# edegens/ptype

Hardware: AMD Instinct MI355X
Metric: messages/sec (higher is better)
Workload: dtype int64; 1 GPU; model=calculator actor (Calculator.Multiply), global_batch=8388608, parallelism=actors sharded over 1 GPU(s), actors=131072, chunks=1, wire=v2, record_bytes=20, reply_bytes=9, client_batch=SoA (actor u32, A i64, B i64), hip_graph=True, steps_per_graph=1, placement=random, delivery=mailbox, mailbox_slots=131072, mailbox_ring_bytes=1344380288, mailbox_record_bytes=8

## Files before the change

### ptype_amd/csrc/hip/mailbox_sort.hip

```cpp
#include "mailbox_sort_dev.hpp"

namespace ptype {

template <int MODE>
__global__ __launch_bounds__(kST) void mbx_count_kernel(SortIn in, uint32_t log_s, uint32_t* __restrict__ hist,
                                                        uint32_t* __restrict__ gsum, uint32_t* __restrict__ rw) {
  __shared__ uint32_t cnt[kMboxSortMaxShards];
  const uint32_t S = 1u << log_s;
  const uint32_t v = virt_block(blockIdx.x, in.G);
  for (uint32_t s = threadIdx.x; s < S; s += kST) cnt[s] = 0;
  __syncthreads();
  const uint32_t t0 = v * in.tpb, t1 = min(t0 + in.tpb, in.tiles);
  uint32_t a[kSK];
  if (t0 < t1) load_actors(in, t0, a);
  for (uint32_t t = t0; t < t1; ++t) {
    int r[kSK];
    uint32_t mb[kSK];
    resolve_k<MODE>(in, a, r, mb);
    if (t + 1 < t1) load_actors(in, t + 1, a);
#pragma unroll
    for (int k = 0; k < kSK; ++k) {
      const int64_t i = tile_index(t, k);
      const bool ok = r[k] == in.rank_self && mb[k] < kMaxMbox;
      if (i < in.M) rw[i] = ok ? mb[k] : kNoSlot;
// ... 108 lines not shown
      }
      const uint32_t off = wcnt(w, sh[k]) + wr[k];
      if (off >= room[sh[k]]) {
        if (spill) {
          ++n_spill;
          sidx[i] = kSpillSlot;
          continue;
        }
        ++n_ovf;
        if (wsidx) sidx[i] = kNoSlot;
        write_status(rv, origin, kStatusOverflow);
        continue;
      }
      const int64_t x0 = v0[k], x1 = v1[k], x2 = v2[k];
      const uint32_t mt = meth[k];
      const uint64_t slot = slot_at(mv, sh[k], base[sh[k]] + off);
      if (wsidx) sidx[i] = (uint32_t)slot;
      if (mt < 128u && fits_i32(x0) && fits_i32(x1) && x2 == 0) {
        *reinterpret_cast<u32x4*>(rec_a(mv, slot)) =
            u32x4{origin | kCompactMark, mb[k] | (mt << 24), (uint32_t)x0, (uint32_t)x1};
      } else {
        const uint32_t fl = x2 != 0 ? (uint32_t)kFlagA2 : 0u;
        *reinterpret_cast<u32x4*>(rec_a(mv, slot)) =
            u32x4{origin | kCompactMark, mb[k] | kCompactLong, (mt & 0xffffu) | (fl << 16), 0u};
        *reinterpret_cast<u32x4*>(rec_b(mv, slot)) =
            u32x4{(uint32_t)x0, (uint32_t)((uint64_t)x0 >> 32), (uint32_t)x1, (uint32_t)((uint64_t)x1 >> 32)};
        if (fl) mv.a2[slot] = x2;
      }
      ++n_enq;
    }
    if (tinfo) {
      for (uint32_t s = threadIdx.x; s < S; s += kST) {
        const uint32_t r0 = wcnt(0, s), rr = run[s];
        const uint32_t cc = r0 >= room[s] ? 0u : min(rr - r0, room[s] - r0);
        tinfo[(size_t)t * 2 * S + s] = (uint32_t)(base[s] + r0) + shard_rot(mv, s);
        tinfo[(size_t)t * 2 * S + S + s] = cc | (rr > room[s] ? kRunSpilled : 0u);
      }
    }
    __syncthreads();
  }
  block_add_stats(mv.stats, n_enq, kMbEnqueued, n_ovf, kMbOverflow, n_miss, kMbNoActor);
  if (spill) {
    __syncthreads();
    block_add_stats(mv.stats, n_spill, kMbSpilled, 0, -1, 0, -1);
  }
}

template <int = 0>
__global__ __launch_bounds__(256) void mbx_presence_kernel(const uint8_t* __restrict__ dirr, uint32_t n_dir,
                                                           int rank_self, uint32_t* __restrict__ pres) {
  const uint32_t wi = blockIdx.x * 256u + threadIdx.x;
  if (wi >= pres_words(n_dir)) return;
  alignas(16) uint8_t b[16];
  if (wi * 16 + 16 <= n_dir) {
    *reinterpret_cast<uint4*>(b) = *reinterpret_cast<const uint4*>(dirr + (size_t)wi * 16);
  } else {
#pragma unroll
    for (uint32_t j = 0; j < 16; ++j) b[j] = wi * 16 + j < n_dir ? dirr[wi * 16 + j] : kRankMissing;
  }
  uint32_t w = 0;
#pragma unroll
  for (uint32_t j = 0; j < 16; ++j) {
    const uint32_t st = b[j] == (uint8_t)rank_self ? 1u : b[j] == kRankFallback ? 2u : 0u;
    w |= st << (2 * j);
  }
  pres[wi] = w;
}

template <int MODE, bool A2, bool MC>
__global__ __launch_bounds__(kST) void mbx_onesweep_kernel(SortIn in, MboxView mv, unsigned long long* __restrict__ desc,
                                                           unsigned* __restrict__ tctr, uint32_t* __restrict__ gsum,
                                                           uint32_t* __restrict__ sidx, uint32_t* __restrict__ tinfo,
                                                           uint32_t* __restrict__ rw, ReplyView rv, bool spill,
                                                           bool all_sidx, bool reserve) {
  extern __shared__ __align__(16) unsigned char smem_os[];
  (void)onesweep_tile<MODE, A2, MC>(in, mv, desc, tctr, gsum, sidx, tinfo, rw, rv, spill, all_sidx, smem_os, reserve);
}

__host__ __device__ constexpr size_t persist_lds_bytes(uint32_t S) {
  return (size_t)S * (8 + 4 + 2 * 4 + 2 * 4 * (kST / kWave));
}

template <int = 0>
__global__ __launch_bounds__(kST) void mbx_persist_sort_kernel(SortIn in, MboxView mv, uint32_t* __restrict__ sidx,
                                                               uint32_t* __restrict__ tinfo, uint32_t* __restrict__ rw,
                                                               ReplyView rv) {
  constexpr int SK = kSK;
  extern __shared__ __align__(16) unsigned char smem_ps[];
  const uint32_t S = 1u << mv.log_s;
  unsigned long long* base = reinterpret_cast<unsigned long long*>(smem_ps);
  uint32_t* room = reinterpret_cast<uint32_t*>(base + S);
  uint32_t* pre2 = room + S;
  uint32_t* wcnt2 = pre2 + 2 * S;
  uint32_t* lpres = reinterpret_cast<uint32_t*>(smem_ps + ((persist_lds_bytes(S) + 15) & ~(size_t)15));
  __shared__ uint32_t tmax[3];
  __shared__ uint32_t vote[2];
  const unsigned w = threadIdx.x / kWave, lane = lane_id();
  const uint32_t G = gridDim.x, T = in.tiles;
  uint32_t first = blockIdx.x, stride = G, n = blockIdx.x < T ? (T - blockIdx.x + G - 1) / G : 0u;
  if (G >= 8 && (G & 7) == 0 && (T & 7) == 0) {
    const uint32_t j = blockIdx.x >> 3, T8 = T >> 3;
    stride = G >> 3;
    first = (blockIdx.x & 7) * T8 + j;
    n = j < T8 ? (T8 - j + stride - 1) / stride : 0u;
  }
  if (n == 0) return;
  stage_pres(in, lpres);
  for (uint32_t s = threadIdx.x; s < S; s += kST) {
    uint64_t tl;
    room[s] = os_ring_room(mv, s, tl);
    base[s] = tl;
  }
  if (threadIdx.x < 3) tmax[threadIdx.x] = 0;
  if (threadIdx.x < 2) vote[threadIdx.x] = 0;
  for (uint32_t s = lane; s < S; s += kWave) wcnt2[w * S + s] = 0;
  __syncthreads();
  const uint32_t w8 = in.rec8 ? *in.r8w : 0u;
  const bool maxima = in.rec8 || in.recw;
  uint32_t n_enq = 0, n_ovf = 0, n_miss = 0, n_spill = 0;
  uint32_t nx[SK];
  int64_t v0[SK], v1[SK];
  PackedRanks<SK> wrp;
  {
    uint32_t a[SK], wr[SK];
    int r[SK];
    const bool full = tile_is_full<SK>(in, first);
    load_actors<SK>(in, first, a);
    load_args_tile<SK>(in, first, full, v0, v1);
    os_resolve<4, SK>(in, lpres, a, r, nx);
    os_rank<SK>(in, mv.log_s, first, r, nx, wcnt2 + w * S, wr);
#pragma unroll
    for (int k = 0; k < SK / 2; ++k) wrp.p[k] = wr[2 * k] | (wr[2 * k + 1] << 16);
  }
  __syncthreads();
  uint32_t rc = 0, rx = 0;
  if (threadIdx.x < S) {
    rc = os_wave_offsets(wcnt2, S, threadIdx.x);
    rx = os_reserve(mv, threadIdx.x, rc);
  }
  for (uint32_t it = 0; it < n; ++it) {
    const uint32_t t = first + it * stride, b = it & 1;
    uint32_t* pre = pre2 + b * S;
    uint32_t* wcnt_all = wcnt2 + b * (kST / kWave) * S;
    const bool full = tile_is_full<SK>(in, t);
    uint32_t mb[SK];
#pragma unroll
    for (int k = 0; k < SK; ++k) mb[k] = nx[k];
    const bool more = it + 1 < n;
    const bool full_next = more && tile_is_full<SK>(in, t + stride);
    if (more) load_actors<SK>(in, t + stride, nx);
    os_loads_in<SK>(v0, v1, nx);
    int sp = 0;
    if (threadIdx.x < S) {
      const uint32_t s = threadIdx.x;
      pre[s] = rx;
      sp = os_run_info(mv, tinfo, t, S, s, base[s], room[s], rx, rc);
    }
    const uint32_t escm = os_fields<SK>(in, w8, mb, v0, v1, tmax);
    sp |= escm != 0;
    if (__any(sp) && lane == 0) vote[b] = 1u;
    __syncthreads();
    const bool tile_spill = __builtin_amdgcn_readfirstlane((int)vote[b]) != 0;
    if (threadIdx.x == 0) {
      if (tile_spill) tinfo[(size_t)t * 2 * S + S] |= kRunSpilled;
      if (maxima) {
        (void)atomicExch(&in.r8max[t], tmax[0] | (tmax[1] << 8) | (tmax[2] << 16));
        tmax[0] = tmax[1] = tmax[2] = 0;
      }
    }
#pragma unroll
    for (int k = 0; k < SK; ++k) {
      const int64_t i = tile_index<SK>(t, k);
      if (!full && i >= in.M) continue;
      os_store_msg<SK>(in, mv, rv, i, base, room, pre, wcnt_all + w * S, mb[k], wrp[k], v0[k], v1[k], 0, in.method_uniform,
                       (escm >> k) & 1u, w8, true, tile_spill, sidx, rw, n_enq, n_ovf, n_miss, n_spill);
    }
    if (more) {
      load_args_tile<SK>(in, t + stride, full_next, v0, v1);
      uint32_t* wnext = wcnt2 + (b ^ 1) * (kST / kWave) * S;
      for (uint32_t s = lane; s < S; s += kWave) wnext[w * S + s] = 0;
      uint32_t a[SK], wr[SK];
      int r[SK];
#pragma unroll
      for (int k = 0; k < SK; ++k) a[k] = nx[k];
      os_resolve<4, SK>(in, lpres, a, r, nx);
      os_rank<SK>(in, mv.log_s, t + stride, r, nx, wnext + w * S, wr);
#pragma unroll
      for (int k = 0; k < SK / 2; ++k) wrp.p[k] = wr[2 * k] | (wr[2 * k + 1] << 16);
      __syncthreads();
      if (threadIdx.x == 0) vote[b] = 0u;
      if (threadIdx.x < S) {
        rc = os_wave_offsets(wnext, S, threadIdx.x);
        rx = os_reserve(mv, threadIdx.x, rc);
      }
    }
  }
  block_add_stats(mv.stats, n_enq, kMbEnqueued, n_ovf, kMbOverflow, n_miss, kMbNoActor);
  __syncthreads();
  block_add_stats(mv.stats, n_spill, kMbSpilled, 0, -1, 0, -1);
}

template <int FIXED>
__global__ __launch_bounds__(kST) void mbx_drain_msg_kernel(MboxView mv, SortIn in, const uint32_t* __restrict__ sidx,
                                                            const uint32_t* __restrict__ rw,
                                                            int64_t* __restrict__ state, uint32_t n_state,
                                                            uint64_t delay_ticks, OutboxView ob, ReplyView rv,
                                                            uint32_t* __restrict__ gsum, uint32_t ngroups,
                                                            unsigned* __restrict__ ticket, unsigned* __restrict__ tctr) {
  unsigned long long done = 0, failed = 0, holes = 0;
  const uint32_t v = virt_block(blockIdx.x, in.G);
  const uint32_t t0 = v * in.tpb, t1 = min(t0 + in.tpb, in.tiles);
  for (uint32_t t = t0; t < t1; ++t)
    drain_tile_msg<FIXED>(mv, in, t, sidx, rw, state, n_state, delay_ticks, ob, rv, done, failed, holes);
  block_add_stats(mv.stats, done, kMbProcessed, failed, kMbFailed, holes, kMbHoles);
  __shared__ bool last;
  if (threadIdx.x == 0) last = last_block_ticket(ticket);
  __syncthreads();
  if (last) {
    const uint32_t S = 1u << mv.log_s;
    for (uint32_t s = threadIdx.x; s < S; s += kST) epoch_commit(mv, s, epoch_sum(mv, gsum, ngroups, S, s));
    if (threadIdx.x == 0) tctr[1] += 1u;
  }
}

template <int FIXED, bool NARROW, int RF, int SK = kSK>
__global__ __launch_bounds__(kST, (NARROW && FIXED) ? 8 : 1) void mbx_drain_ring_kernel(MboxView mv, SortIn in, const uint32_t* __restrict__ tinfo,
                                                             const uint32_t* __restrict__ sidx,
                                                             const uint32_t* __restrict__ rw,
                                                             int64_t* __restrict__ state, uint32_t n_state,
                                                             uint64_t delay_ticks, OutboxView ob, ReplyView rv,
                                                             uint32_t* __restrict__ gsum, uint32_t ngroups,
                                                             unsigned* __restrict__ ticket, unsigned* __restrict__ tctr,
                                                             uint32_t* __restrict__ r8host) {
  extern __shared__ __align__(16) unsigned char smem_rd[];
  const uint32_t S = 1u << mv.log_s;
  DrainCounts dc;
  const uint32_t t = virt_block(blockIdx.x, gridDim.x);
  if (t < in.tiles)
    dc = drain_ring_tile<FIXED, NARROW, false, RF, SK>(mv, in, t, tinfo, sidx, rw, state, n_state, delay_ticks, ob,
                                                       rv, smem_rd);
  block_add_stats(mv.stats, dc.done, kMbProcessed, dc.failed, kMbFailed, dc.holes, kMbHoles);
  __shared__ bool last;
  if (threadIdx.x == 0) last = last_block_ticket(ticket);
  __syncthreads();
  if (last) {
    for (uint32_t s = threadIdx.x; s < S; s += kST) epoch_commit(mv, s, epoch_sum(mv, gsum, ngroups, S, s));
    if (threadIdx.x == 0) tctr[1] += 1u;
    if constexpr (RF != 0) rec8_next(in, const_cast<uint32_t*>(in.r8w), r8host, in.tiles);
  }
}


static const Variant<decltype(mbx_count_kernel<0>)> kCount[] = {
    MBX_ROW(vkey(0), 0, mbx_count_kernel<0>),
    MBX_ROW(vkey(1), 0, mbx_count_kernel<1>),
    MBX_ROW(vkey(2), 0, mbx_count_kernel<2>),
};
static const Variant<decltype(mbx_scatter_kernel<false, false>)> kScatter[] = {
// ... 291 lines not shown
```

### ptype_amd/csrc/hip/mailbox_sort_dev.hpp

```cpp
#pragma once
#include <algorithm>
#include <string>
#include <type_traits>
#include <vector>

#include "mailbox.hpp"
#include "mailbox_dev.hpp"
#include "route_common.hpp"
#include "sort_common.hpp"
#include "tune.hpp"

namespace ptype {

namespace {
constexpr uint32_t kCompactMark = 0x80000000u;
constexpr uint32_t kCompactLong = 0x80000000u;
}

constexpr uint32_t kNoSlot = 0xffffffffu;
constexpr uint32_t kSpillSlot = 0xfffffffeu;
constexpr uint32_t kRunSpilled = 0x80000000u;
constexpr int kWaitVmcnt0 = 0x0f70;

__host__ __device__ constexpr size_t onesweep_lds_bytes(uint32_t S) { return (size_t)S * (8 + 4 + 4 + 4 * (kST / kWave)); }
// ... 79 lines not shown
}

__device__ __forceinline__ void stage_pres(const SortIn& in, uint32_t* lpres) {
  const uint32_t nw = pres_words(in.n_dir);
  for (uint32_t w = threadIdx.x * 4; w < nw; w += blockDim.x * 4)
    *reinterpret_cast<uint4*>(lpres + w) = *reinterpret_cast<const uint4*>(in.pres + w);
}
template <int SK>
__device__ __forceinline__ void resolve_pres(const SortIn& in, const uint32_t* lpres, const uint32_t (&a)[SK],
                                             int (&r)[SK], uint32_t (&mb)[SK]) {
#pragma unroll
  for (int k = 0; k < SK; ++k) {
    mb[k] = a[k];
    if (a[k] < in.n_dir) {
      const uint32_t st = (lpres[a[k] >> 4] >> ((a[k] & 15) * 2)) & 3u;
      r[k] = st == 1 ? in.rank_self : -1;
      if (st == 2) lookup_entry(in.table, in.mask, actor_key(a[k]), r[k], mb[k]);
    } else if (a[k] != 0xffffffffu) {
      lookup_entry(in.table, in.mask, actor_key(a[k]), r[k], mb[k]);
    } else {
      r[k] = -1;
    }
  }
}

template <int MODE, int SK>
__device__ __forceinline__ void os_resolve(const SortIn& in, const uint32_t* lpres, const uint32_t (&a)[SK], int (&r)[SK],
                                           uint32_t (&mb)[SK]) {
  if constexpr (MODE == 4) resolve_pres<SK>(in, lpres, a, r, mb);
  else resolve_k<MODE, SK>(in, a, r, mb);
}

template <int SK>
__device__ __forceinline__ void os_rank(const SortIn& in, uint32_t log_s, uint32_t t, const int (&r)[SK],
                                        uint32_t (&mb)[SK], uint32_t* wrow, uint32_t (&wr)[SK]) {
  const uint32_t S = 1u << log_s;
#pragma unroll
  for (int k = 0; k < SK; ++k) {
    const bool ok = tile_index<SK>(t, k) < in.M && r[k] == in.rank_self && mb[k] < kMaxMbox;
    if (!ok) mb[k] = kNoSlot;
    const uint32_t sh = mb[k] & (S - 1);
    const uint64_t peers = match_bits(sh, log_s, __ballot(ok));
    const unsigned below = mbcnt64(peers);
    const int leader = peers ? __builtin_ctzll(peers) : 0;
    unsigned old = 0;
    if (ok && below == 0) {
      old = wrow[sh];
      wrow[sh] = old + (unsigned)__popcll(peers);
    }
    wr[k] = (unsigned)__shfl((int)old, leader) + below;
  }
}

__device__ __forceinline__ uint32_t os_wave_offsets(uint32_t* wcnt_all, uint32_t S, uint32_t s) {
  uint32_t c = 0;
#pragma unroll
  for (int ww = 0; ww < kST / kWave; ++ww) {
    const uint32_t x = wcnt_all[ww * S + s];
    wcnt_all[ww * S + s] = c;
    c += x;
  }
  return c;
}
__device__ __forceinline__ uint32_t os_reserve(const MboxView& mv, uint32_t s, uint32_t c) {
  return c ? atomicAdd(&mv.resv[s * kResvStride], c) : 0u;
}
__device__ __forceinline__ uint32_t os_ring_room(const MboxView& mv, uint32_t s, uint64_t& tl) {
  const uint64_t Q = 1ull << mv.log_q;
  tl = *ctr_tail(mv, s);
  const uint64_t hd = *ctr_head(mv, s);
  const uint64_t free = hd + Q > tl ? hd + Q - tl : 0;
  return (uint32_t)(free < 0xffffffffull ? free : 0xffffffffull);
}
__device__ __forceinline__ int os_run_info(const MboxView& mv, uint32_t* __restrict__ tinfo, uint32_t t, uint32_t S,
                                           uint32_t s, uint64_t tl, uint32_t rm, uint64_t excl, uint32_t c) {
  if (tinfo) {
    const uint32_t cc = excl >= rm ? 0u : (uint32_t)min((uint64_t)c, rm - excl);
    tinfo[(size_t)t * 2 * S + s] = (uint32_t)(tl + excl) + shard_rot(mv, s);
    tinfo[(size_t)t * 2 * S + S + s] = cc | (excl + c > rm ? kRunSpilled : 0u);
  }
  return excl + c > rm;
}

template <int SK>
__device__ __forceinline__ uint32_t os_fields(const SortIn& in, uint32_t w8, const uint32_t (&mb)[SK],
                                              const int64_t (&v0)[SK], const int64_t (&v1)[SK], uint32_t* tmax) {
  uint32_t escm = 0;
  if (!(in.rec8 || in.recw)) return escm;
  uint64_t or_m = 0, or_0 = 0, or_1 = 0;
  const uint32_t wm = w8 & 0xffu, w0 = (w8 >> 8) & 0xffu, w1 = (w8 >> 16) & 0xffu;
#pragma unroll
  for (int k = 0; k < SK; ++k) {
    if (mb[k] == kNoSlot) continue;
    const uint64_t z0 = ((uint64_t)v0[k] << 1) ^ (uint64_t)(v0[k] >> 63);
    const uint64_t z1 = ((uint64_t)v1[k] << 1) ^ (uint64_t)(v1[k] >> 63);
    or_m |= mb[k], or_0 |= z0, or_1 |= z1;
    if (in.rec8 && ((mb[k] >> wm) != 0 || (z0 >> w0) != 0 || (z1 >> w1) != 0)) escm |= 1u << k;
  }
  const uint32_t bm = wave_max_u32(bitlen64(or_m)), b0 = wave_max_u32(bitlen64(or_0)),
                 b1 = wave_max_u32(bitlen64(or_1));
  if (lane_id() == 0) {
    atomicMax(&tmax[0], bm);
    atomicMax(&tmax[1], b0);
    atomicMax(&tmax[2], b1);
  }
  return escm;
}

template <int SK>
__device__ __forceinline__ void os_loads_in(const int64_t (&v0)[SK], const int64_t (&v1)[SK], const uint32_t (&nx)[SK]) {
#pragma unroll
  for (int k = 0; k < SK; ++k) asm volatile("" ::"v"(v0[k]), "v"(v1[k]), "v"(nx[k]));
}

template <int SK>
struct PackedRanks {
  uint32_t p[SK / 2];
  __device__ __forceinline__ uint32_t operator[](int k) const { return (p[k >> 1] >> ((k & 1) * 16)) & 0xffffu; }
};

template <int SK, typename CT>
__device__ __forceinline__ void os_store_msg(const SortIn& in, const MboxView& mv, const ReplyView& rv, int64_t i,
                                             const unsigned long long* base, const uint32_t* room, const uint32_t* pre,
                                             const uint32_t* wrow, uint32_t mbk, uint32_t wrk, int64_t x0, int64_t x1,
                                             int64_t x2, uint32_t mt, bool esc, uint32_t w8, bool spill, bool wsidx,
                                             uint32_t* __restrict__ sidx, uint32_t* __restrict__ rw, CT& n_enq, CT& n_ovf,
                                             CT& n_miss, CT& n_spill) {
  const uint32_t S = 1u << mv.log_s;
  const uint32_t origin = in.origin_base + (uint32_t)i;
  if (mbk == kNoSlot) {
    ++n_miss;
    if (wsidx) sidx[i] = kNoSlot;
    write_status(rv, origin, kStatusNoActor);
    return;
  }
  const uint32_t sh = mbk & (S - 1);
  const uint32_t off = pre[sh] + wrow[sh] + wrk;
  if (off >= room[sh] || (esc && spill)) {
    if (spill) {
      ++n_spill;
      sidx[i] = kSpillSlot;
      rw[i] = mbk;
      return;
    }
    ++n_ovf;
    if (wsidx) sidx[i] = kNoSlot;
    write_status(rv, origin, kStatusOverflow);
    return;
  }
  const uint64_t slot = slot_at(mv, sh, base[sh] + off);
  if (wsidx) sidx[i] = (uint32_t)slot;
  if (in.recw) {
    *reinterpret_cast<u32x4*>(rec_a(mv, slot)) =
        u32x4{(uint32_t)x0, (uint32_t)((uint64_t)x0 >> 32), (uint32_t)x1, (uint32_t)((uint64_t)x1 >> 32)};
    rec_place(mv)[slot] = (uint16_t)(i & ((kST * SK) - 1));
  } else if (in.rec8 && esc) {
    reinterpret_cast<uint64_t*>(mv.rec)[slot] = (uint64_t)(i & ((kST * SK) - 1)) | (1ull << 63);
    *reinterpret_cast<u32x4*>(in.r8esc + 2 * slot) =
        u32x4{(uint32_t)x0, (uint32_t)((uint64_t)x0 >> 32), mbk, 0u};
  } else if (in.rec8) {
    const uint32_t wm = w8 & 0xffu, w0 = (w8 >> 8) & 0xffu;
    const uint64_t z0 = ((uint64_t)x0 << 1) ^ (uint64_t)(x0 >> 63);
    const uint64_t z1 = ((uint64_t)x1 << 1) ^ (uint64_t)(x1 >> 63);
    reinterpret_cast<uint64_t*>(mv.rec)[slot] =
        (uint64_t)(i & ((kST * SK) - 1)) | ((uint64_t)mbk << 12) | (z0 << (12 + wm)) | (z1 << (12 + wm + w0));
  } else if (mt < 128u && fits_i32(x0) && fits_i32(x1) && x2 == 0) {
    *reinterpret_cast<u32x4*>(rec_a(mv, slot)) =
        u32x4{origin | kCompactMark, mbk | (mt << 24), (uint32_t)x0, (uint32_t)x1};
  } else {
    const uint32_t fl = x2 != 0 ? (uint32_t)kFlagA2 : 0u;
    *reinterpret_cast<u32x4*>(rec_a(mv, slot)) =
        u32x4{origin | kCompactMark, mbk | kCompactLong, (mt & 0xffffu) | (fl << 16), 0u};
    *reinterpret_cast<u32x4*>(rec_b(mv, slot)) =
        u32x4{(uint32_t)x0, (uint32_t)((uint64_t)x0 >> 32), (uint32_t)x1, (uint32_t)((uint64_t)x1 >> 32)};
    if (fl) mv.a2[slot] = x2;
  }
  ++n_enq;
}

template <int MODE, bool A2, bool MC, int SK = kSK>
__device__ __forceinline__ uint32_t onesweep_tile(const SortIn& in, const MboxView& mv, unsigned long long* __restrict__ desc,
                                                  unsigned* __restrict__ tctr, uint32_t* __restrict__ gsum,
                                                  uint32_t* __restrict__ sidx, uint32_t* __restrict__ tinfo,
                                                  uint32_t* __restrict__ rw, const ReplyView& rv, bool spill,
                                                  bool all_sidx, unsigned char* smem_os, bool reserve = false) {
  const uint32_t S = 1u << mv.log_s;
  unsigned long long* base = reinterpret_cast<unsigned long long*>(smem_os);
  uint32_t* room = reinterpret_cast<uint32_t*>(base + S);
  uint32_t* pre = room + S;
  uint32_t* wcnt_all = pre + S;
  auto wcnt = [&](unsigned ww, uint32_t sh) -> uint32_t& { return wcnt_all[ww * S + sh]; };
  __shared__ uint32_t tile_s;
  __shared__ uint32_t tmax[3];
  const unsigned w = threadIdx.x / kWave, lane = lane_id();
  if (threadIdx.x < 3) tmax[threadIdx.x] = 0;
  const uint32_t tag = epoch_tag(tctr[1]);
  if (threadIdx.x == 0 && !reserve) {
    const uint32_t t = atomicAdd(&tctr[0], 1u);
    if (t == in.tiles - 1) atomicExch(&tctr[0], 0u);
    tile_s = t;
  }
  for (uint32_t s = lane; s < S; s += kWave) wcnt(w, s) = 0;
// ... 189 lines not shown
      x.a2 = in.a2 ? in.a2[i] : 0;
    } else if constexpr (RF == 1) {
      x = decode_rec8<FRESH, SK>(ha[k], in, w8, in.origin_base + t * (kST * SK));
    } else if constexpr (RF == 2) {
      x = decode_wide(ha[k], in, 0u);
    } else {
      u32x4 hb = {0u, 0u, 0u, 0u};
      int64_t a2v = 0;
      if (rec_is_long(ha[k])) {
        const u32x4* bp = reinterpret_cast<const u32x4*>(rec_b(mv, sl[k]));
        hb = FRESH ? __builtin_nontemporal_load(bp) : *bp;
        if (((ha[k].z >> 16) & kFlagA2) && mv.a2) a2v = FRESH ? __builtin_nontemporal_load(mv.a2 + sl[k]) : mv.a2[sl[k]];
      }
      x = decode_sorted(ha[k], hb, a2v);
    }
    const uint32_t origin = in.origin_base + (uint32_t)tile_index<SK>(t, k);
    if (!x.valid) {
      ++holes;
      write_status(rv, origin, kStatusNotDelivered);
      continue;
    }
    MsgRecord m;
    m.actor = x.mb;
    m.method = (uint16_t)(FIXED ? FIXED : x.method);
    m.flags = (uint16_t)x.flags;
    m.a0 = x.a0, m.a1 = x.a1, m.a2 = x.a2;
    const ReplyRecord rr = run_handler(m, state, n_state, delay_ticks, ob);
    failed += rr.status != kStatusOk;
    write_reply(rv, origin, rr);
    ++done;
  }
}

template <typename OwnT>
struct RunLds {
  uint32_t* bias;
  uint32_t* excl;
  OwnT* owner;
};

template <typename OwnT>
__device__ __forceinline__ uint32_t load_tile_runs(const MboxView& mv, const uint32_t* __restrict__ tinfo, uint32_t t,
                                                   const RunLds<OwnT>& L, int& spill) {
  __shared__ uint32_t wsum[kST / kWave];
  __shared__ uint32_t total_s;
  const uint32_t S = 1u << mv.log_s;
  const unsigned w = threadIdx.x / kWave, lane = lane_id();
  const uint32_t per = (S + kST - 1) / kST, s0 = threadIdx.x * per, s1 = min(S, s0 + per);
  uint32_t cnt[2] = {0u, 0u};
  uint32_t mine = 0;
  int sp = 0;
  for (uint32_t s = s0, q = 0; s < s1; ++s, ++q) {
    const uint32_t cw = tinfo[(size_t)t * 2 * S + S + s];
    sp |= (cw & kRunSpilled) != 0;
    cnt[q] = cw & ~kRunSpilled;
    mine += cnt[q];
    L.bias[s] = tinfo[(size_t)t * 2 * S + s];
  }
  const uint32_t incl = wave_incl_scan(mine);
  if (lane == kWave - 1) wsum[w] = incl;
  spill = __syncthreads_or(sp);
  uint32_t acc = incl - mine;
  for (unsigned ww = 0; ww < w; ++ww) acc += wsum[ww];
  if (threadIdx.x == kST - 1) total_s = acc + mine;
  for (uint32_t s = s0, q = 0; s < s1; ++s, ++q) {
    L.excl[s] = acc;
    L.bias[s] -= acc;
    for (uint32_t j = acc; j < acc + cnt[q]; ++j) L.owner[j] = (OwnT)s;
    acc += cnt[q];
  }
  __syncthreads();
  return total_s;
}

constexpr uint8_t kAbsent = 0xff;
__host__ __device__ constexpr size_t ring_drain_lds_bytes(uint32_t S, size_t tile = kSTile) {
  return S <= 256 ? tile * (8 + 1) + (size_t)S * 8 : tile * (8 + 2 + 1) + (size_t)S * 8;
}

struct DrainCounts {
  unsigned long long done = 0, failed = 0, holes = 0;
};

template <int FIXED, bool NARROW, bool FRESH, int RF = 0, int SK = kSK>
__device__ __forceinline__ DrainCounts drain_ring_tile(MboxView mv, SortIn in, uint32_t t,
                                                       const uint32_t* __restrict__ tinfo,
                                                       const uint32_t* __restrict__ sidx,
                                                       const uint32_t* __restrict__ rw, int64_t* __restrict__ state,
                                                       uint32_t n_state, uint64_t delay_ticks, OutboxView ob,
                                                       ReplyView rv, unsigned char* smem_rd) {
  unsigned long long done = 0, failed = 0, holes = 0;
  using OwnT = typename std::conditional<NARROW, uint8_t, uint16_t>::type;
  const uint32_t S = 1u << mv.log_s;
  int64_t* sval = reinterpret_cast<int64_t*>(smem_rd);
  RunLds<OwnT> L;
  L.bias = reinterpret_cast<uint32_t*>(sval + (kST * SK));
  L.excl = L.bias + S;
  L.owner = reinterpret_cast<OwnT*>(L.excl + S);
  uint8_t* sst = NARROW ? reinterpret_cast<uint8_t*>(L.owner) : reinterpret_cast<uint8_t*>(L.owner + (kST * SK));
  const uint64_t i0 = (uint64_t)t * (kST * SK);
  const uint32_t n_t = (uint32_t)min((uint64_t)(kST * SK), (uint64_t)in.M - i0);
  if constexpr (!NARROW)
    for (uint32_t j = threadIdx.x; j < (kST * SK); j += kST) sst[j] = kAbsent;
  int spill = 0;
  const uint32_t T = load_tile_runs(mv, tinfo, t, L, spill);
  if (spill) {
    drain_tile_msg<FIXED, FRESH, RF, SK>(mv, in, t, sidx, rw, state, n_state, delay_ticks, ob, rv, done, failed, holes);
    return DrainCounts{done, failed, holes};
  }
  const uint64_t sbase_mask = (1ull << mv.log_q) - 1;
  using RecT = typename std::conditional<RF == 1, uint64_t, u32x4>::type;
  const uint32_t w8 = RF == 1 ? *in.r8w : 0u;
  RecT ha[SK];
  uint32_t sl[SK];
  uint16_t pl[SK];
#pragma unroll
  for (int k = 0; k < SK; ++k) {
    const uint32_t j = (uint32_t)k * kST + threadIdx.x;
    sl[k] = kNoSlot;
    if (j < T) {
      const uint32_t s = L.owner[j];
      sl[k] = (uint32_t)(((uint64_t)s << mv.log_q) | ((L.bias[s] + j) & sbase_mask));
      if constexpr (RF == 1) {
        const uint64_t* rp = reinterpret_cast<const uint64_t*>(mv.rec) + sl[k];
        ha[k] = FRESH ? __builtin_nontemporal_load(rp) : *rp;
      } else {
        const u32x4* rp = reinterpret_cast<const u32x4*>(rec_a(mv, sl[k]));
        ha[k] = FRESH ? __builtin_nontemporal_load(rp) : *rp;
        if constexpr (RF == 2) {
          const uint16_t* pp = rec_place(mv) + sl[k];
          pl[k] = FRESH ? __builtin_nontemporal_load(pp) : *pp;
        }
      }
    }
  }
  if constexpr (NARROW) {
    __syncthreads();
    for (uint32_t j = threadIdx.x; j < (kST * SK); j += kST) sst[j] = kAbsent;
    __syncthreads();
  }
#pragma unroll
  for (int k = 0; k < SK; ++k) {
    if (sl[k] == kNoSlot) continue;
    SortRec x;
    if constexpr (RF == 1) {
      x = decode_rec8<FRESH, SK>(ha[k], in, w8, in.origin_base + (uint32_t)i0);
    } else if constexpr (RF == 2) {
      x = decode_wide(ha[k], in, in.origin_base + (uint32_t)i0 + pl[k]);
    } else {
      u32x4 hb = {0u, 0u, 0u, 0u};
      int64_t a2v = 0;
      if (rec_is_long(ha[k])) {
        const u32x4* bp = reinterpret_cast<const u32x4*>(rec_b(mv, sl[k]));
        hb = FRESH ? __builtin_nontemporal_load(bp) : *bp;
        if (((ha[k].z >> 16) & kFlagA2) && mv.a2) a2v = FRESH ? __builtin_nontemporal_load(mv.a2 + sl[k]) : mv.a2[sl[k]];
      }
      x = decode_sorted(ha[k], hb, a2v);
    }
    const uint32_t local = x.origin - in.origin_base - (uint32_t)i0;
    if (!x.valid || local >= n_t) {
      ++holes;
      continue;
    }
    MsgRecord m;
    m.actor = x.mb;
    m.method = (uint16_t)(FIXED ? FIXED : x.method);
    m.flags = (uint16_t)x.flags;
    m.a0 = x.a0, m.a1 = x.a1, m.a2 = x.a2;
    const ReplyRecord rr = run_handler(m, state, n_state, delay_ticks, ob);
    failed += rr.status != kStatusOk;
    sval[local] = rr.value;
    sst[local] = (uint8_t)rr.status;
    ++done;
  }
  __builtin_amdgcn_s_waitcnt(kWaitVmcnt0);
  __syncthreads();
  uint8_t rst[SK];
  int64_t rval[SK];
#pragma unroll
  for (int k = 0; k < SK; ++k) {
    const uint32_t j = (uint32_t)k * kST + threadIdx.x;
    rst[k] = j < n_t ? sst[j] : kAbsent;
    rval[k] = sval[j];
  }
// ... 67 lines not shown
```

Before: 65.13 billion msg/s.

## Add lean rec8 store and drain paths for small-shard stateless mailbox rings

Adds a specialized enqueue path in the persistent sort kernel for the 8-byte record case with few shards and small rings. It precomputes per-shard rotated bases, skips the general os_store_msg bookkeeping, and packs records with 32-bit zigzag shifts. On the drain side it adds a matching lean drain that resolves run slots with wave readlane instead of an LDS owner table and decodes with alignbit. It also defers the per-element escape check behind a wave-wide OR and pins the kernel to 4 waves per EU. These changes target ALU and LDS overhead per message, at the cost of much more specialized code and a possibly lower occupancy cap.

```diff
diff --git a/ptype_amd/csrc/hip/mailbox_sort.hip b/ptype_amd/csrc/hip/mailbox_sort.hip
--- a/ptype_amd/csrc/hip/mailbox_sort.hip
+++ b/ptype_amd/csrc/hip/mailbox_sort.hip
@@ -214,9 +214,9 @@
 }
 
 template <int = 0>
-__global__ __launch_bounds__(kST) void mbx_persist_sort_kernel(SortIn in, MboxView mv, uint32_t* __restrict__ sidx,
-                                                               uint32_t* __restrict__ tinfo, uint32_t* __restrict__ rw,
-                                                               ReplyView rv) {
+__global__ __launch_bounds__(kST) __attribute__((amdgpu_waves_per_eu(4, 4)))
+void mbx_persist_sort_kernel(SortIn in, MboxView mv, uint32_t* __restrict__ sidx, uint32_t* __restrict__ tinfo,
+                             uint32_t* __restrict__ rw, ReplyView rv) {
   constexpr int SK = kSK;
   extern __shared__ __align__(16) unsigned char smem_ps[];
   const uint32_t S = 1u << mv.log_s;
@@ -227,6 +227,7 @@
   uint32_t* lpres = reinterpret_cast<uint32_t*>(smem_ps + ((persist_lds_bytes(S) + 15) & ~(size_t)15));
   __shared__ uint32_t tmax[3];
   __shared__ uint32_t vote[2];
+  __shared__ uint32_t brot[kStatelessShards];
   const unsigned w = threadIdx.x / kWave, lane = lane_id();
   const uint32_t G = gridDim.x, T = in.tiles;
   uint32_t first = blockIdx.x, stride = G, n = blockIdx.x < T ? (T - blockIdx.x + G - 1) / G : 0u;
@@ -242,6 +243,7 @@
     uint64_t tl;
     room[s] = os_ring_room(mv, s, tl);
     base[s] = tl;
+    if (s < kStatelessShards) brot[s] = (uint32_t)tl + shard_rot(mv, s);
   }
   if (threadIdx.x < 3) tmax[threadIdx.x] = 0;
   if (threadIdx.x < 2) vote[threadIdx.x] = 0;
@@ -249,6 +251,8 @@
   __syncthreads();
   const uint32_t w8 = in.rec8 ? *in.r8w : 0u;
   const bool maxima = in.rec8 || in.recw;
+  const bool lean = in.rec8 && !in.recw && tinfo != nullptr && rv.slots == nullptr && S <= kStatelessShards &&
+                    rings_small(mv);
   uint32_t n_enq = 0, n_ovf = 0, n_miss = 0, n_spill = 0;
   uint32_t nx[SK];
   int64_t v0[SK], v1[SK];
@@ -288,7 +292,7 @@
       pre[s] = rx;
       sp = os_run_info(mv, tinfo, t, S, s, base[s], room[s], rx, rc);
     }
-    const uint32_t escm = os_fields<SK>(in, w8, mb, v0, v1, tmax);
+    const uint32_t escm = os_fields<SK, true>(in, w8, mb, v0, v1, tmax);
     sp |= escm != 0;
     if (__any(sp) && lane == 0) vote[b] = 1u;
     __syncthreads();
@@ -300,12 +304,36 @@
         tmax[0] = tmax[1] = tmax[2] = 0;
       }
     }
-#pragma unroll
-    for (int k = 0; k < SK; ++k) {
-      const int64_t i = tile_index<SK>(t, k);
-      if (!full && i >= in.M) continue;
-      os_store_msg<SK>(in, mv, rv, i, base, room, pre, wcnt_all + w * S, mb[k], wrp[k], v0[k], v1[k], 0, in.method_uniform,
-                       (escm >> k) & 1u, w8, true, tile_spill, sidx, rw, n_enq, n_ovf, n_miss, n_spill);
+    if (lean && !tile_spill) {
+      uint32_t* wpos = wcnt_all + w * S;
+      if (lane < S) wpos[lane] += pre[lane] + brot[lane];
+      __builtin_amdgcn_wave_barrier();
+      if (threadIdx.x < S) n_enq += rc;
+      const Rec8Fast f8 = rec8_fast(w8);
+      const uint32_t place0 = w * (SK * kWave) + lane;
+      if (f8.ok) {
+#pragma unroll
+        for (int k = 0; k < SK; ++k) {
+          const int64_t i = tile_index<SK>(t, k);
+          if (!full && i >= in.M) continue;
+          os_store_lean<SK, true>(in, mv, rv, i, place0 + k * kWave, wpos, mb[k], wrp[k], v0[k], v1[k], f8, w8, n_miss);
+        }
+      } else {
+#pragma unroll
+        for (int k = 0; k < SK; ++k) {
+          const int64_t i = tile_index<SK>(t, k);
+          if (!full && i >= in.M) continue;
+          os_store_lean<SK, false>(in, mv, rv, i, place0 + k * kWave, wpos, mb[k], wrp[k], v0[k], v1[k], f8, w8, n_miss);
+        }
+      }
+    } else {
+#pragma unroll
+      for (int k = 0; k < SK; ++k) {
+        const int64_t i = tile_index<SK>(t, k);
+        if (!full && i >= in.M) continue;
+        os_store_msg<SK>(in, mv, rv, i, base, room, pre, wcnt_all + w * S, mb[k], wrp[k], v0[k], v1[k], 0, in.method_uniform,
+                         (escm >> k) & 1u, w8, true, tile_spill, sidx, rw, n_enq, n_ovf, n_miss, n_spill);
+      }
     }
     if (more) {
       load_args_tile<SK>(in, t + stride, full_next, v0, v1);
diff --git a/ptype_amd/csrc/hip/mailbox_sort_dev.hpp b/ptype_amd/csrc/hip/mailbox_sort_dev.hpp
--- a/ptype_amd/csrc/hip/mailbox_sort_dev.hpp
+++ b/ptype_amd/csrc/hip/mailbox_sort_dev.hpp
@@ -185,7 +185,7 @@
   return excl + c > rm;
 }
 
-template <int SK>
+template <int SK, bool OR_FIRST = false>
 __device__ __forceinline__ uint32_t os_fields(const SortIn& in, uint32_t w8, const uint32_t (&mb)[SK],
                                               const int64_t (&v0)[SK], const int64_t (&v1)[SK], uint32_t* tmax) {
   uint32_t escm = 0;
@@ -198,7 +198,17 @@
     const uint64_t z0 = ((uint64_t)v0[k] << 1) ^ (uint64_t)(v0[k] >> 63);
     const uint64_t z1 = ((uint64_t)v1[k] << 1) ^ (uint64_t)(v1[k] >> 63);
     or_m |= mb[k], or_0 |= z0, or_1 |= z1;
-    if (in.rec8 && ((mb[k] >> wm) != 0 || (z0 >> w0) != 0 || (z1 >> w1) != 0)) escm |= 1u << k;
+    if constexpr (!OR_FIRST)
+      if (in.rec8 && ((mb[k] >> wm) != 0 || (z0 >> w0) != 0 || (z1 >> w1) != 0)) escm |= 1u << k;
+  }
+  if (OR_FIRST && in.rec8 && ((or_m >> wm) | (or_0 >> w0) | (or_1 >> w1)) != 0) {
+#pragma unroll
+    for (int k = 0; k < SK; ++k) {
+      if (mb[k] == kNoSlot) continue;
+      const uint64_t z0 = ((uint64_t)v0[k] << 1) ^ (uint64_t)(v0[k] >> 63);
+      const uint64_t z1 = ((uint64_t)v1[k] << 1) ^ (uint64_t)(v1[k] >> 63);
+      if ((mb[k] >> wm) != 0 || (z0 >> w0) != 0 || (z1 >> w1) != 0) escm |= 1u << k;
+    }
   }
   const uint32_t bm = wave_max_u32(bitlen64(or_m)), b0 = wave_max_u32(bitlen64(or_0)),
                  b1 = wave_max_u32(bitlen64(or_1));
@@ -221,6 +231,63 @@
   uint32_t p[SK / 2];
   __device__ __forceinline__ uint32_t operator[](int k) const { return (p[k >> 1] >> ((k & 1) * 16)) & 0xffffu; }
 };
+
+__device__ __forceinline__ bool rings_small(const MboxView& mv) { return mv.log_s + mv.log_q <= 29; }
+
+struct Rec8Fast {
+  uint32_t s0;
+  uint32_t s1h;
+  uint32_t m0;
+  uint32_t mm;
+  bool ok;
+};
+__device__ __forceinline__ Rec8Fast rec8_fast(uint32_t w8) {
+  const uint32_t wm = w8 & 0xffu, w0 = (w8 >> 8) & 0xffu, w1 = (w8 >> 16) & 0xffu;
+  Rec8Fast f;
+  f.s0 = 12 + wm;
+  f.ok = f.s0 < 32 && w0 >= 1 && w0 <= 32 && w1 <= 32 && f.s0 + w0 >= 32 && f.s0 + w0 < 64;
+  f.s1h = (f.s0 + w0) & 31u;
+  f.m0 = w0 >= 32 ? 0xffffffffu : (1u << (w0 & 31u)) - 1u;
+  f.mm = (1u << (wm & 31u)) - 1u;
+  return f;
+}
+__device__ __forceinline__ uint32_t zigzag32(int64_t x) {
+  const uint32_t lo = (uint32_t)x;
+  return (lo << 1) ^ (uint32_t)((int32_t)lo >> 31);
+}
+__device__ __forceinline__ uint64_t pack_rec8_fast(const Rec8Fast& f, uint32_t place, uint32_t mb, int64_t x0, int64_t x1) {
+  const uint32_t z0 = zigzag32(x0), z1 = zigzag32(x1);
+  const uint32_t lo = place | (mb << 12) | (z0 << f.s0);
+  const uint32_t hi = (z0 >> (32u - f.s0)) | (z1 << f.s1h);
+  return ((uint64_t)hi << 32) | lo;
+}
+
+template <int SK, bool FAST>
+__device__ __forceinline__ void os_store_lean(const SortIn& in, const MboxView& mv, const ReplyView& rv, int64_t i,
+                                              uint32_t place, const uint32_t* wpos, uint32_t mbk, uint32_t wrk,
+                                              int64_t x0, int64_t x1, const Rec8Fast& f, uint32_t w8, uint32_t& n_miss) {
+  if (mbk == kNoSlot) {
+    ++n_miss;
+    const uint32_t origin = in.origin_base + (uint32_t)i;
+    if ((uint64_t)origin < rv.n) {
+      rv.val[origin] = 0;
+      rv.st[origin] = kStatusNoActor;
+    }
+    return;
+  }
+  const uint32_t sh = mbk & ((1u << mv.log_s) - 1u);
+  const uint32_t slot = (sh << mv.log_q) | ((wpos[sh] + wrk) & ((1u << mv.log_q) - 1u));
+  uint64_t rec;
+  if constexpr (FAST) {
+    rec = pack_rec8_fast(f, place, mbk, x0, x1);
+  } else {
+    const uint32_t wm = w8 & 0xffu, w0 = (w8 >> 8) & 0xffu;
+    const uint64_t z0 = ((uint64_t)x0 << 1) ^ (uint64_t)(x0 >> 63);
+    const uint64_t z1 = ((uint64_t)x1 << 1) ^ (uint64_t)(x1 >> 63);
+    rec = (uint64_t)place | ((uint64_t)mbk << 12) | (z0 << (12 + wm)) | (z1 << (12 + wm + w0));
+  }
+  *reinterpret_cast<uint64_t*>(reinterpret_cast<unsigned char*>(mv.rec) + (slot << 3)) = rec;
+}
 
 template <int SK, typename CT>
 __device__ __forceinline__ void os_store_msg(const SortIn& in, const MboxView& mv, const ReplyView& rv, int64_t i,
@@ -576,6 +643,137 @@
   unsigned long long done = 0, failed = 0, holes = 0;
 };
 
+struct Run8Lds {
+  uint32_t bias[kStatelessShards];
+  uint32_t excl[kStatelessShards];
+  uint32_t grp[(kST * kSK) / kWave];
+  uint32_t total, spill;
+};
+template <int SK>
+__device__ __forceinline__ uint32_t load_tile_runs8(const MboxView& mv, const uint32_t* __restrict__ tinfo, uint32_t t,
+                                                    Run8Lds& R, int& spill) {
+  static_assert((kST * SK) / kWave <= kWave && kStatelessShards <= kWave, "one lane per group and per shard");
+  const uint32_t S = 1u << mv.log_s;
+  if (threadIdx.x < kWave) {
+    const uint32_t lane = threadIdx.x;
+    uint32_t cnt = 0, bw = 0;
+    int sp = 0;
+    if (lane < S) {
+      const uint32_t cw = tinfo[(size_t)t * 2 * S + S + lane];
+      sp = (cw & kRunSpilled) != 0;
+      cnt = cw & ~kRunSpilled;
+      bw = tinfo[(size_t)t * 2 * S + lane];
+    }
+    const uint32_t incl = wave_incl_scan(cnt), ex = incl - cnt;
+    if (lane < kStatelessShards) {
+      R.bias[lane] = bw - ex;
+      R.excl[lane] = ex;
+    }
+    const uint32_t jf = lane * kWave, jl = jf + (kWave - 1);
+    uint32_t sf = 0, sl = 0;
+#pragma unroll
+    for (int q = 1; q < (int)kStatelessShards; ++q) {
+      const uint32_t e = (uint32_t)__builtin_amdgcn_readlane((int)ex, q);
+      sf += jf >= e, sl += jl >= e;
+    }
+    if (lane < (kST * SK) / kWave) R.grp[lane] = sf | (sl << 8);
+    const bool any_sp = __any(sp) != 0;
+    if (lane == kWave - 1) R.total = incl, R.spill = any_sp;
+  }
+  __syncthreads();
+  spill = (int)R.spill;
+  return R.total;
+}
+
+template <int FIXED, int SK>
+__device__ __forceinline__ DrainCounts drain_ring_tile_lean(MboxView mv, SortIn in, uint32_t i0, uint32_t n_t, uint32_t T,
+                                                            const Run8Lds& R, int64_t* sval, uint8_t* sst,
+                                                            int64_t* __restrict__ state, uint32_t n_state,
+                                                            uint64_t delay_ticks, OutboxView ob, ReplyView rv) {
+  unsigned long long done = 0, failed = 0, holes = 0;
+  const uint32_t w8 = *in.r8w;
+  const Rec8Fast f = rec8_fast(w8);
+  const uint32_t qmask = (1u << mv.log_q) - 1u;
+  const unsigned char* recs = reinterpret_cast<const unsigned char*>(mv.rec);
+  const uint32_t wv = threadIdx.x / kWave, lane = lane_id();
+  const uint32_t gp = R.grp[(lane & (SK - 1)) * (kST / kWave) + wv];
+  const uint32_t bl = R.bias[lane & (kStatelessShards - 1)];
+  uint64_t ha[SK];
+#pragma unroll
+  for (int k = 0; k < SK; ++k) {
+    const uint32_t j = (uint32_t)k * kST + threadIdx.x;
+    const uint32_t pair = (uint32_t)__builtin_amdgcn_readlane((int)gp, k);
+    const uint32_t sf = pair & 0xffu;
+    uint32_t slot;
+    if (sf == (pair >> 8)) {
+      const uint32_t b = (uint32_t)__builtin_amdgcn_readlane((int)bl, sf);
+      slot = (sf << mv.log_q) | ((b + j) & qmask);
+    } else {
+      uint32_t s = 0;
+#pragma unroll
+      for (uint32_t q = 1; q < kStatelessShards; ++q) s += j >= R.excl[q];
+      slot = (s << mv.log_q) | ((R.bias[s] + j) & qmask);
+    }
+    if (j < T) ha[k] = *reinterpret_cast<const uint64_t*>(recs + (slot << 3));
+  }
+#pragma unroll
+  for (int k = 0; k < SK; ++k) {
+    const uint32_t j = (uint32_t)k * kST + threadIdx.x;
+    if (j >= T) continue;
+    const uint32_t lo = (uint32_t)ha[k], hi = (uint32_t)(ha[k] >> 32);
+    const uint32_t local = lo & ((kST * SK) - 1);
+    if (local >= n_t) {
+      ++holes;
+      continue;
+    }
+    MsgRecord m;
+    m.method = (uint16_t)(FIXED ? FIXED : in.method_uniform);
+    m.flags = 0;
+    m.a2 = 0;
+    if (f.ok) {
+      const uint32_t z0 = __builtin_amdgcn_alignbit(hi, lo, f.s0) & f.m0, z1 = hi >> f.s1h;
+      m.actor = (lo >> 12) & f.mm;
+      m.a0 = (int64_t)(int32_t)((z0 >> 1) ^ (0u - (z0 & 1u)));
+      m.a1 = (int64_t)(int32_t)((z1 >> 1) ^ (0u - (z1 & 1u)));
+    } else {
+      const SortRec x = decode_rec8<false, SK>(ha[k], in, w8, 0u);
+      m.actor = x.mb;
+      m.a0 = x.a0, m.a1 = x.a1;
+    }
+    const ReplyRecord rr = run_handler(m, state, n_state, delay_ticks, ob);
+    failed += rr.status != kStatusOk;
+    sval[local] = rr.value;
+    sst[local] = (uint8_t)rr.status;
+    ++done;
+  }
+  __builtin_amdgcn_s_waitcnt(kWaitVmcnt0);
+  __syncthreads();
+  uint8_t rst[SK];
+  int64_t rval[SK];
+#pragma unroll
+  for (int k = 0; k < SK; ++k) {
+    const uint32_t j = (uint32_t)k * kST + threadIdx.x;
+    rst[k] = j < n_t ? sst[j] : kAbsent;
+    rval[k] = sval[j];
+  }
+  const uint32_t o0 = in.origin_base + i0;
+  const bool whole = (uint64_t)o0 + (kST * SK) <= rv.n && (uint64_t)o0 + (kST * SK) <= 0x100000000ull;
+  int64_t* vb = rv.val + o0;
+  int32_t* sb = rv.st + o0;
+#pragma unroll
+  for (int k = 0; k < SK; ++k) {
+    const uint32_t j = (uint32_t)k * kST + threadIdx.x;
+    if (rst[k] == kAbsent) continue;
+    if (whole) {
+      __builtin_nontemporal_store(rval[k], vb + j);
+      __builtin_nontemporal_store((int32_t)rst[k], sb + j);
+    } else {
+      put_reply_nt(rv, o0 + j, rval[k], rst[k]);
+    }
+  }
+  return DrainCounts{done, failed, holes};
+}
+
 template <int FIXED, bool NARROW, bool FRESH, int RF = 0, int SK = kSK>
 __device__ __forceinline__ DrainCounts drain_ring_tile(MboxView mv, SortIn in, uint32_t t,
                                                        const uint32_t* __restrict__ tinfo,
@@ -594,6 +792,22 @@
   uint8_t* sst = NARROW ? reinterpret_cast<uint8_t*>(L.owner) : reinterpret_cast<uint8_t*>(L.owner + (kST * SK));
   const uint64_t i0 = (uint64_t)t * (kST * SK);
   const uint32_t n_t = (uint32_t)min((uint64_t)(kST * SK), (uint64_t)in.M - i0);
+  constexpr bool kLeanForm = NARROW && RF == 1 && !FRESH;
+  if constexpr (kLeanForm) {
+    if (rv.slots == nullptr && S <= kStatelessShards && rings_small(mv)) {
+      __shared__ Run8Lds R8;
+      for (uint32_t j = threadIdx.x; j < (kST * SK); j += kST) sst[j] = kAbsent;
+      int spill8 = 0;
+      const uint32_t T8 = load_tile_runs8<SK>(mv, tinfo, t, R8, spill8);
+      if (spill8) {
+        drain_tile_msg<FIXED, FRESH, RF, SK>(mv, in, t, sidx, rw, state, n_state, delay_ticks, ob, rv, done, failed,
+                                             holes);
+        return DrainCounts{done, failed, holes};
+      }
+      return drain_ring_tile_lean<FIXED, SK>(mv, in, (uint32_t)i0, n_t, T8, R8, sval, sst, state, n_state, delay_ticks,
+                                             ob, rv);
+    }
+  }
   if constexpr (!NARROW)
     for (uint32_t j = threadIdx.x; j < (kST * SK); j += kST) sst[j] = kAbsent;
   int spill = 0;
```

After: 67.38 billion msg/s (median of 6 runs). +3.5%, better.
